# uguryagmur/RealTimeObjectDetection

Hardware: AMD Instinct MI355X
Metric: frames/sec YOLOv3 608x608 bs=8 (Darknet.forward + write_results; 2 batches in flight, write_results_async on a second stream) (higher is better)
Workload: dtype f16x2-split (3 MFMA products, f32 accumulate); 1 GPU; YOLOv3 cfg 608x608 batch=8 per GPU, split-f16 MFMA conv + fused head + GPU NMS (BASELINE configs[2]); precision=f16s3, tiles=autotune (this run), parallelism=frame-shard x1, in_flight_batches=2, detections_last_step=1699, candidates_last_step=1914, f16_range_overflow=False

## Files before the change

realtimeobjectdetection_amd/csrc/conv_f16s3_common.h:

```cpp
#pragma once
#include "rtod_internal.h"
#include <type_traits>

namespace rtod {

typedef float f32x4 __attribute__((ext_vector_type(4)));
typedef _Float16 f16x8 __attribute__((ext_vector_type(8)));
typedef unsigned int u32x4 __attribute__((ext_vector_type(4)));

constexpr int HBK = 32;
constexpr unsigned OOB = 0x80000000u;


template <int N> __device__ __forceinline__ void vmcnt() {
    static_assert(0 <= N && N <= 63, "vmcnt range");
    asm volatile("s_waitcnt vmcnt(%0)" :: "n"(N) : "memory");
}

template <int OFF = 0> __device__ __forceinline__ u32x4 buffer_load_b128(const __amdgpu_buffer_rsrc_t rsrc, unsigned voffset, unsigned soffset) {
    u32x4 v;
    asm volatile("buffer_load_dwordx4 %0, %1, %2, %3 offen offset:%4" : "=v"(v) : "v"(voffset), "s"(rsrc), "s"(soffset), "n"(OFF) : "memory");
    return v;
}

// ... 169 lines not shown
        if (kg == 1) return;
#pragma unroll
        for (int i = 0; i < TM; ++i)
#pragma unroll
            for (int j = 0; j < TN; ++j) {
                const f32x4 o = T[base + (i * TN + j) * 64];
#pragma unroll
                for (int e = 0; e < 4; ++e) acc[i][j][e] += o[e];
            }
    }
    float amax = 0.f;
    _Float16* const oh = reinterpret_cast<_Float16*>(a.out) + a.out_coff;
    const _Float16* const rh = reinterpret_cast<const _Float16*>(a.res) + a.res_coff;
#pragma unroll
    for (int P = 0; P < NP; ++P) {
        const int c0 = cbase + 32 * P + 8 * lh;
        const bool cok = c0 < a.Cout;
        const int cc = cok ? c0 : 0;
        f16x8 rq_h[RES ? TM : 1], rq_l[RES ? TM : 1];
        if constexpr (RES) {
#pragma unroll
            for (int i = 0; i < TM; ++i) {
                const int m = mrow[i];
                const bool ok = m >= 0 && cok;
                const _Float16* q = rh + (int64_t)(ok ? m : 0) * 2 * a.res_ldc + cc;
                rq_h[i] = ok ? *reinterpret_cast<const f16x8*>(q) : f16x8{0, 0, 0, 0, 0, 0, 0, 0};
                rq_l[i] = ok ? *reinterpret_cast<const f16x8*>(q + a.res_ldc) : f16x8{0, 0, 0, 0, 0, 0, 0, 0};
            }
        }
        f32x4 iv0 = *reinterpret_cast<const f32x4*>(a.inv_scale + cc), iv1 = *reinterpret_cast<const f32x4*>(a.inv_scale + cc + 4);
        f32x4 bs0 = *reinterpret_cast<const f32x4*>(a.bias + cc), bs1 = *reinterpret_cast<const f32x4*>(a.bias + cc + 4);
#pragma unroll
        for (int i = 0; i < TM; ++i) {
            const int m = mrow[i];
            f16x8 ph, pl;
#pragma unroll
            for (int e = 0; e < 8; ++e) {
                const float s = e < 4 ? acc[i][2 * P][e] : acc[i][2 * P + 1][e - 4];
                float v = s * ((e < 4 ? iv0[e] : iv1[e - 4]) * SPLIT_SCALE) + (e < 4 ? bs0[e] : bs1[e - 4]) * SPLIT_SCALE;
                if (a.leaky) v = v > 0.f ? v : v * 0.1f;
                if constexpr (RES) v += (float)rq_h[i][e] + (float)rq_l[i][e];
                _Float16 h, l;
                split_f16(v, h, l, amax);
                ph[e] = h; pl[e] = l;
            }
            if (m >= 0 && cok) {
                _Float16* q = oh + (int64_t)m * 2 * a.out_ldc + c0;
                store_act16(q, ph, false);
                store_act16(q + a.out_ldc, pl, false);
            }
        }
    }
    split_overflow_report(a.ovf, amax);
}

constexpr int epi_row_group(int bm, int wm, int rg_max) {
    int best = wm;
    for (int r = wm; r <= bm && r <= rg_max; r += wm) if (bm % r == 0) best = r;
    return best;
}


template <int BM, int BN, int WM, int WN, int NT, int EPI, int SMEM_BYTES, int KG = 1, bool PRE = false, bool F16 = false, bool RAW = false>
__device__ __forceinline__ void conv_f16s3_epilogue(const ConvArgs& a, f32x4 (&acc)[WM / 16][WN / 16], unsigned char* smem,
                                                    int bm, int bn, int tid, int wm, int wn, int lr, int lh, int M, int kg = 0,
                                                    const float* pre_bias = nullptr, const float* pre_inv = nullptr) {
    constexpr int MT = 16, TM = WM / MT, TN = WN / MT;
    constexpr bool PW = EPI == EPI_SPLIT_PW || EPI == EPI_SPLIT_RES_PW;
    constexpr bool RES = EPI == EPI_SPLIT_RES || EPI == EPI_SPLIT_RES_PW;
    static_assert(!(F16 && PW), "plain-f16 plans host no pointwise conv");
    static_assert(!RAW || (EPI == EPI_SPLIT && !F16), "raw-sum instances: no shortcut, decode, hosted pointwise conv or plain-f16 store");
    constexpr int TS = PW ? BN + 4 : BN;
    constexpr int T2S = PW_MAX_COUT + 4;
    constexpr int RG_MAX = SMEM_BYTES / ((TS + (PW ? T2S : 0)) * 4);
    constexpr int RG = epi_row_group(BM, WM, RG_MAX);
    static_assert(RG >= WM && BM % RG == 0, "epilogue row group");
    static_assert(RG * (TS + (PW ? T2S : 0)) * 4 <= SMEM_BYTES, "epilogue tile exceeds the kernel's LDS");
    float* T = reinterpret_cast<float*>(smem);
    const int hw = a.Ho * a.Wo;
#ifdef RTOD_DIAG
    const bool st_plain = (a.dbg & 8) != 0;
#else
    constexpr bool st_plain = false;
#endif
    float amax = 0.f;
    constexpr int PWK = PW_MAX_K / 32;
    f16x8 b2h[PW ? PWK : 1], b2l[PW ? PWK : 1];
    float bias2 = 0.f, inv2 = 0.f;
    int pw_n2t = 1, pw_j = 0;
    if constexpr (PW) {
        pw_n2t = a.pw_cout / 16;
        pw_j = (tid >> 6) % pw_n2t;
        const int n2 = pw_j * 16 + (tid & 15);
        const _Float16* w2h = a.pw_wh + (int64_t)n2 * 32 + ((tid & 63) >> 4) * 8;
        const _Float16* w2l = a.pw_wl + (int64_t)n2 * 32 + ((tid & 63) >> 4) * 8;
#pragma unroll
        for (int ks = 0; ks < PWK; ++ks) {
            const bool ok = ks * 32 < a.pw_k;
            b2h[ks] = ok ? *reinterpret_cast<const f16x8*>(w2h + (int64_t)ks * a.pw_npad * 32) : f16x8{0, 0, 0, 0, 0, 0, 0, 0};
            b2l[ks] = ok ? *reinterpret_cast<const f16x8*>(w2l + (int64_t)ks * a.pw_npad * 32) : f16x8{0, 0, 0, 0, 0, 0, 0, 0};
        }
        bias2 = a.pw_bias[n2] * SPLIT_SCALE; inv2 = a.pw_inv_scale[n2] * SPLIT_SCALE;
    }
    const float escale = (EPI == EPI_DECODE || RAW) ? 1.0f : SPLIT_SCALE;
    constexpr int GPR_ = BN / 8;
    constexpr int NG = (RG * GPR_ + NT - 1) / NT;
#pragma unroll 1
    for (int rg = 0; rg < BM; rg += RG) {
        float bias_j[TN], inv_j[TN];
#pragma unroll
        for (int j = 0; j < TN; ++j) {
            if constexpr (PRE) { bias_j[j] = pre_bias[j]; inv_j[j] = pre_inv[j]; }
            else epi_col_params(a, bn * BN + wn * WN + j * MT + lr, bias_j[j], inv_j[j]);
        }
        f16x8 rq_h[RES ? NG : 1], rq_l[RES ? NG : 1];
        if constexpr (RES) {
            const _Float16* rh0 = reinterpret_cast<const _Float16*>(a.res) + a.res_coff + bn * BN;
#pragma unroll
            for (int i = 0; i < NG; ++i) {
                const int g = tid + i * NT;
                const int r = g / GPR_, c8 = (g - r * GPR_) * 8;
                const int m = bm * BM + rg + r;
                const bool ok = g < RG * GPR_ && m < M && bn * BN + c8 < a.Cout;
                const _Float16* q = rh0 + (int64_t)(ok ? m : 0) * 2 * a.res_ldc + (ok ? c8 : 0);
                const f16x8 th = *reinterpret_cast<const f16x8*>(q);
                rq_h[i] = ok ? th : f16x8{0, 0, 0, 0, 0, 0, 0, 0};
                if constexpr (!F16) {
                    const f16x8 tl = *reinterpret_cast<const f16x8*>(q + a.res_ldc);
                    rq_l[i] = ok ? tl : f16x8{0, 0, 0, 0, 0, 0, 0, 0};
                }
            }
        }
#define EPI_WAVE_IN_PASS (RG == BM || (wm * WM >= rg && wm * WM < rg + RG))
#define EPI_TILE_IN_PASS(i) true
#define EPI_TILE_ROW(i) (wm * WM - rg + (i) * MT)
#include "conv_f16s3_epi_transpose.inc"
#undef EPI_WAVE_IN_PASS
#undef EPI_TILE_IN_PASS
#undef EPI_TILE_ROW
        __syncthreads();
        if constexpr (EPI == EPI_DECODE) {
            constexpr int RSTEP = NT / BN > 0 ? NT / BN : 1;
            static_assert(NT % BN == 0 || BN % NT == 0, "decode mapping");
            for (int nl = tid % BN; nl < BN; nl += NT) {
                const int n = bn * BN + nl;
                if (n >= a.Cout) continue;
                const int an = n / a.dec.attrs, c = n - an * a.dec.attrs;
                const bool is_wh = (c == 2 || c == 3) && !a.dec.train;
                const bool is_raw = (c == 2 || c == 3) && a.dec.train;
                const float anc = (c == 2 ? a.dec.aw[an] : a.dec.ah[an]);
                const int r0 = (NT >= BN) ? tid / BN : 0;
                int m = bm * BM + rg + r0;
                const int b = m / hw;
                int cell = m - b * hw;
                int gy = cell / a.dec.GW, gx = cell - gy * a.dec.GW;
                float* op = a.out + (int64_t)b * a.dec.img_stride + a.dec.head_off + (int64_t)cell * a.Cout + n;
                const int64_t row_step = (int64_t)RSTEP * a.Cout;
                const int64_t img_fix = a.dec.img_stride - (int64_t)hw * a.Cout;
                if (a.dec.v5) {
                    for (int r = r0; r < RG && m < M; r += RSTEP, m += RSTEP) {
                        const float sg = __builtin_amdgcn_rcpf(1.0f + __expf(-T[r * TS + nl]));
                        float o = sg;
                        if (c < 2) o = ((sg * 2.0f - 0.5f) + (float)(c == 0 ? gx : gy)) * a.dec.stride;
                        else if (c < 4) { const float t2 = sg * 2.0f; o = (t2 * t2) * anc; }
                        *op = o;
                        op += row_step; cell += RSTEP; gx += RSTEP;
                        while (gx >= a.dec.GW) { gx -= a.dec.GW; ++gy; }
                        while (cell >= hw) { cell -= hw; gy -= a.dec.GH; op += img_fix; }
                    }
                } else
                for (int r = r0; r < RG && m < M; r += RSTEP, m += RSTEP) {
                    const float v = T[r * TS + nl];
                    float o;
                    if (is_raw) o = v;
                    else {
                        const float ex = __expf(is_wh ? v : -v);
                        if (is_wh) o = (ex * anc) * a.dec.stride;
                        else {
                            o = __builtin_amdgcn_rcpf(1.0f + ex);
                            if (c < 2 && !a.dec.train) o = (o + (float)(c == 0 ? gx : gy)) * a.dec.stride;
                        }
                    }
                    *op = o;
                    op += row_step; cell += RSTEP; gx += RSTEP;
                    while (gx >= a.dec.GW) { gx -= a.dec.GW; ++gy; }
                    while (cell >= hw) { cell -= hw; gy -= a.dec.GH; op += img_fix; }
                }
            }
        } else {
            constexpr int GPR = GPR_;
            _Float16* oh = reinterpret_cast<_Float16*>(a.out) + a.out_coff + bn * BN;
#pragma unroll
            for (int gi = 0; gi < NG; ++gi) {
                const int g = tid + gi * NT;
                if (g >= RG * GPR) continue;
                const int r = g / GPR, c8 = (g - r * GPR) * 8;
                const int m = bm * BM + rg + r;
                if (m >= M || bn * BN + c8 >= a.Cout) continue;
                const f32x4 v0 = *reinterpret_cast<const f32x4*>(T + r * TS + c8);
                const f32x4 v1 = *reinterpret_cast<const f32x4*>(T + r * TS + c8 + 4);
                if constexpr (RAW) {
                    float* rp = a.raw_out + (int64_t)m * a.raw_ld + bn * BN + c8;
                    *reinterpret_cast<f32x4*>(rp) = v0;
                    *reinterpret_cast<f32x4*>(rp + 4) = v1;
                    continue;
                }
                float v[8] = {v0[0], v0[1], v0[2], v0[3], v1[0], v1[1], v1[2], v1[3]};
                if constexpr (RES) {
                    epi_add_shortcut8<F16>(v, rq_h[gi], rq_l[gi]);
                    if constexpr (PW) {
                        *reinterpret_cast<f32x4*>(T + r * TS + c8) = f32x4{v[0], v[1], v[2], v[3]};
                        *reinterpret_cast<f32x4*>(T + r * TS + c8 + 4) = f32x4{v[4], v[5], v[6], v[7]};
                    }
                }
                f16x8 ph, pl;
                epi_split8<F16>(v, ph, pl, amax);
                epi_store8<F16>(oh + (int64_t)m * 2 * a.out_ldc + c8, a.out_ldc, ph, pl, st_plain);
            }
            if constexpr (PW) {
                __syncthreads();
                float* T2 = T + RG * TS;
                const int lane = tid & 63, wave = tid >> 6;
                const int lr16 = lane & 15, lh16 = lane >> 4;
                const int k2s = a.pw_k / 32;
                const int n2 = pw_j * 16 + lr16;
                for (int sl = wave / pw_n2t; sl < RG / 16; sl += (NT / 64) / pw_n2t) {
                    f32x4 acc2 = {0.f, 0.f, 0.f, 0.f};
                    const float* trow = T + (sl * 16 + lr16) * TS + lh16 * 8;
#pragma unroll
                    for (int ks = 0; ks < PWK; ++ks) {
                        if (ks < k2s) {
                            const f32x4 x0 = *reinterpret_cast<const f32x4*>(trow + ks * 32);
                            const f32x4 x1 = *reinterpret_cast<const f32x4*>(trow + ks * 32 + 4);
                            f16x8 ah, al;
#pragma unroll
                            for (int e = 0; e < 8; ++e) {
                                const float x = e < 4 ? x0[e] : x1[e - 4];
                                const _Float16 h = (_Float16)x;
                                ah[e] = h; al[e] = (_Float16)(x - (float)h);
                            }
                            acc2 = __builtin_amdgcn_mfma_f32_16x16x32_f16(al, b2h[ks], acc2, 0, 0, 0);
// ... 39 lines not shown
```

realtimeobjectdetection_amd/csrc/conv_pwd_f16s3.hip:

```cpp
#include "conv_bandd_common.h"

namespace rtod {

template <int BM, int NW, int NST, int MINW, int EPI>
__global__ __launch_bounds__(NW * 64, MINW)
void conv_pwd_f16s3_kernel(const ConvArgs a, const int grid_m, const int grid_n) {
    constexpr bool F16 = epi_f16(EPI);
    constexpr int LB = F16 ? 2 : 4, LP = F16 ? 1 : 2;
    constexpr int BN = NW * 32, NT = NW * 64, TM = BM / 16, TN = 2;
    constexpr int SLAB = BM * 256;
    constexpr int NP = BM / 8;
    constexpr int NPP = (NP + NW - 1) / NW;
    static_assert(BM % 16 == 0 && NPP >= 1 && NPP <= 8, "slab pieces per wave");
    static_assert(NST >= 2 && NST <= 4, "ring depth");
    constexpr int RG = BM * BN * 4 <= 32768 ? BM : (BM / 2) * BN * 4 <= 32768 ? BM / 2 : BM / 4;
    constexpr int WAIT_B = 2 * LB + LP * NPP;
    constexpr int WAIT_SLAB = 2 * LB + (NST - 2) * (LP * NPP + 2 * LB);
    constexpr int WAIT_SLAB_PRO = 2 * LB + (NST - 2) * LP * NPP;

    extern __shared__ __attribute__((aligned(16))) unsigned char smem[];
    const int nwg = grid_m * grid_n;
    int bid = blockIdx.x;
    if (!a.xcd_by_n) bid = xcd_remap(bid, nwg);
    const int bm = bid / grid_n, bn = bid - bm * grid_n;
    const int tid = (int)threadIdx.x;
    const int wave = __builtin_amdgcn_readfirstlane(tid >> 6), lane = tid & 63;
    const int lr = lane & 15, lh = lane >> 4;
    const int M = a.B * a.Hi * a.Wi;
    const int m0 = bm * BM;
    const unsigned PS = (unsigned)a.in_ldc * 4u;
    const unsigned lo_plane = (unsigned)a.in_ldc * 2u;

    const __amdgpu_buffer_rsrc_t rs_a = buffer_rsrc(a.in, a.in_bytes);
    const __amdgpu_buffer_rsrc_t rs_wh = buffer_rsrc(a.w_hi, a.w_bytes);
    const __amdgpu_buffer_rsrc_t rs_wl = buffer_rsrc(a.w_lo, a.w_bytes);
    const unsigned lds0 = (unsigned)(size_t)smem;
    const int NS = a.Cin / 64;

    unsigned dma_vo[NPP];
#pragma unroll
    for (int k = 0; k < NPP; ++k) {
        const int p = wave + k * NW;
        const int r = lane >> 3;
        const int m = m0 + p * 8 + r;
        dma_vo[k] = (p < NP && m < M) ? (unsigned)m * PS + (unsigned)(a.in_coff + (((lane & 7) ^ r) << 3)) * 2u : OOB;
    }
    auto dma_slab = [&](int js) __attribute__((always_inline)) {
        const bool live = js < NS;
        const unsigned soff = (unsigned)js * 128u;
        const unsigned base = lds0 + (unsigned)((js % NST) * SLAB);
#pragma unroll
        for (int k = 0; k < NPP; ++k) {
            const int p = wave + k * NW;
            const unsigned dst = p < NP ? base + (unsigned)((p >> 1) * 4096 + (p & 1) * 1024) : lds0 + (unsigned)(NST * SLAB);
            if constexpr (F16) lds_dma(rs_a, live ? dma_vo[k] : OOB, soff, dst);
// ... 34 lines not shown
        if constexpr (!F16) l = *reinterpret_cast<lds_f16x8*>((unsigned)(o + 4096 * i + 2048));
    };

#pragma unroll
    for (int s = 0; s < NST - 1; ++s) dma_slab(s);
    load_b(0, Bq[0]);
    load_b(1, Bq[1]);

    __builtin_amdgcn_s_setprio(2);
    auto slab_body = [&](int j, auto par_c) __attribute__((always_inline)) {
        constexpr int par = decltype(par_c)::value;
        asm volatile("" : "+v"(xq0), "+v"(xq1));
        if (j < NST - 1) vmcnt<WAIT_SLAB_PRO>(); else vmcnt<WAIT_SLAB>();
        __builtin_amdgcn_sched_barrier(0);
        __builtin_amdgcn_s_barrier();
        dma_slab(j + NST - 1);
        const int slotoff = (int)lds0 + (j % NST) * SLAB;
        read_unit(0, 0, slotoff, Ah[0], Al[0]);
        read_unit(1 / TM, 1 % TM, slotoff, Ah[1], Al[1]);
        __builtin_amdgcn_sched_barrier(0);
#pragma unroll
        for (int u = 0; u < 2 * TM; ++u) {
            const int q = u / TM, i = u % TM;
            if (i == 0) {
                if (q == 0) load_b(2 * j + 2, Bq[(2 * par + 2) % 4]); else load_b(2 * j + 3, Bq[(2 * par + 3) % 4]);
                vmcnt<WAIT_B>();
                if (q == 0) tie_bset<F16>(Bq[2 * par]); else tie_bset<F16>(Bq[2 * par + 1]);
                __builtin_amdgcn_sched_barrier(0);
            }
            if (u + 2 < 2 * TM) read_unit((u + 2) / TM, (u + 2) % TM, slotoff, Ah[(u + 2) % 3], Al[(u + 2) % 3]);
            const f16x8 ah = Ah[u % 3], al = Al[u % 3];
#pragma unroll
            for (int jn = 0; jn < TN; ++jn) {
                const f16x8 bh = __builtin_bit_cast(f16x8, Bq[2 * par + q][jn][0]);
                if constexpr (F16) { acc[i][jn] = __builtin_amdgcn_mfma_f32_16x16x32_f16(ah, bh, acc[i][jn], 0, 0, 0); continue; }
                const f16x8 bl = __builtin_bit_cast(f16x8, Bq[2 * par + q][jn][1]);
                acc[i][jn] = __builtin_amdgcn_mfma_f32_16x16x32_f16(al, bh, acc[i][jn], 0, 0, 0);
                acc[i][jn] = __builtin_amdgcn_mfma_f32_16x16x32_f16(ah, bl, acc[i][jn], 0, 0, 0);
                acc[i][jn] = __builtin_amdgcn_mfma_f32_16x16x32_f16(ah, bh, acc[i][jn], 0, 0, 0);
            }
            __builtin_amdgcn_sched_barrier(0);
        }
    };
#pragma unroll 1
    for (int j = 0; j < NS; j += 2) {
        slab_body(j, std::integral_constant<int, 0>{});
        if (j + 1 < NS) slab_body(j + 1, std::integral_constant<int, 1>{});
    }
    vmcnt<0>();
    tie_bset<F16>(Bq[0]); tie_bset<F16>(Bq[1]); tie_bset<F16>(Bq[2]); tie_bset<F16>(Bq[3]);
    __builtin_amdgcn_sched_barrier(0);
    __builtin_amdgcn_s_setprio(0);

    bandd_epilogue<BM, BN, BM, 32, NT, RG, epi_kind(EPI) == EPI_SPLIT_RES, 1, F16, epi_raw(EPI)>(a, acc, smem, bm, bn, tid, 0, wn, lr, lh, M, 0);
}

template <int BM, int NW, int NST, int MINW>
static int launch_pwd(const ConvArgs& a, hipStream_t s) {
    constexpr int BN = NW * 32, NT = NW * 64;
    constexpr int RG = BM * BN * 4 <= 32768 ? BM : (BM / 2) * BN * 4 <= 32768 ? BM / 2 : BM / 4;
    const int M = a.B * a.Ho * a.Wo;
    const int gm = (M + BM - 1) / BM, gn = (a.Cout + BN - 1) / BN;
    ConvArgs ax = a;
    ax.xcd_by_n = (gn % 8 == 0 && (int64_t)a.Cout * a.K > (int64_t)M * a.Cin) ? 1 : 0;
    constexpr int ring_bytes = NST * BM * 256 + ((BM / 8) % NW ? 4096 : 0), epi_bytes = RG * BN * 4;
    constexpr int lds = ring_bytes > epi_bytes ? ring_bytes : epi_bytes;
    static_assert(lds <= 160 * 1024, "LDS");
    const int fe = a.f16 ? 1 : 0;
    auto k_res = fe ? conv_pwd_f16s3_kernel<BM, NW, NST, MINW, EPI_SPLIT_RES | EPI_F16> : conv_pwd_f16s3_kernel<BM, NW, NST, MINW, EPI_SPLIT_RES>;
    auto k_plain = fe ? conv_pwd_f16s3_kernel<BM, NW, NST, MINW, EPI_SPLIT | EPI_F16> : conv_pwd_f16s3_kernel<BM, NW, NST, MINW, EPI_SPLIT>;
    auto k_raw = conv_pwd_f16s3_kernel<BM, NW, NST, MINW, EPI_SPLIT | EPI_RAW>;
    if constexpr (lds > 64 * 1024) {
        static std::atomic<unsigned long long> attr_done[3] = {{0}, {0}, {0}};
        if (a.raw_out) { if (int rc = lds_opt_in(attr_done[2], lds, "conv_pwd_f16s3", k_raw)) return rc; }
        else if (int rc = lds_opt_in(attr_done[fe], lds, "conv_pwd_f16s3", k_res, k_plain)) return rc;
    }
    if (a.raw_out) {
        hipLaunchKernelGGL(k_raw, dim3(gm * gn), dim3(NT), lds, s, ax, gm, gn);
        return hip_fail(hipGetLastError(), "conv_pwd_f16s3 launch");
    }
    if (a.res) hipLaunchKernelGGL(k_res, dim3(gm * gn), dim3(NT), lds, s, ax, gm, gn);
    else hipLaunchKernelGGL(k_plain, dim3(gm * gn), dim3(NT), lds, s, ax, gm, gn);
    return hip_fail(hipGetLastError(), "conv_pwd_f16s3 launch");
}

#define RTOD_PWD_TILES(X) \
    X(0, 64, 4, 3, 3) X(1, 32, 4, 3, 3) X(2, 128, 4, 3, 1) X(3, 64, 8, 3, 1) X(4, 64, 4, 2, 3) X(5, 32, 4, 4, 3) X(6, 96, 4, 2, 3) X(7, 96, 4, 3, 2) X(8, 48, 4, 3, 3) X(9, 48, 4, 4, 3) X(10, 64, 2, 2, 4)

#define RTOD_X_INFO(idx, bm, nw, nst, minw) {bm, nw * 32, "conv_pwd_f16s3<" #bm "x" #nw "w,r" #nst ">"},
static const ConvVariantInfo kPwdModes[PWD_MODES] = { RTOD_PWD_TILES(RTOD_X_INFO) };
#undef RTOD_X_INFO
const ConvVariantInfo& conv_pwd_mode_info(int idx) { return kPwdModes[idx < 0 || idx >= PWD_MODES ? 0 : idx]; }

bool conv_pwd_supported(int ksize, int stride, int pad, int cin) { return ksize == 1 && stride == 1 && pad == 0 && cin >= 64 && cin % 64 == 0; }

int conv_pwd_kernel_name(int idx, int epi, char* buf, size_t len) {
#define RTOD_X_NAME(i, bm, nw, nst, minw) \
    if (idx == i) return snprintf(buf, len, "void rtod::conv_pwd_f16s3_kernel<" #bm ", " #nw ", " #nst ", " #minw ", %d>(rtod::ConvArgs, int, int)", epi);
    RTOD_PWD_TILES(RTOD_X_NAME)
#undef RTOD_X_NAME
    return -1;
}

int launch_conv_pwd_f16s3(const ConvArgs& a, int idx, hipStream_t s) {
    if (int rc = check_split_conv_args(a, "launch_conv_pwd", true)) return rc;
    if (!conv_pwd_supported(a.kh, a.stride, a.pad, a.Cin) || a.kw != 1 || a.Ho != a.Hi || a.Wo != a.Wi || a.dec.enabled || a.pw_wh) {
        set_error("launch_conv_pwd: unsupported shape (k=%d s=%d pad=%d Cin=%d)", a.kh, a.stride, a.pad, a.Cin); return RTOD_E_ARG;
    }
    if (a.in_ldc % 8 || a.in_coff % 8 || a.K != a.Kpad || a.K != a.Cin || a.Npad % 128) { set_error("launch_conv_pwd: bad view / K"); return RTOD_E_ARG; }
    if (a.raw_out && (a.f16 || a.res)) { set_error("launch_conv_pwd: a raw-sum launch carries no shortcut and no plain-f16 store"); return RTOD_E_ARG; }
    if (a.raw_out && a.raw_ld != a.Npad) { set_error("launch_conv_pwd: raw-sum rows are Npad floats in this family (raw_ld %d, Npad %d)", a.raw_ld, a.Npad); return RTOD_E_ARG; }
    switch (idx) {
#define RTOD_X_CASE(i, bm, nw, nst, minw) case i: return launch_pwd<bm, nw, nst, minw>(a, s);
        RTOD_PWD_TILES(RTOD_X_CASE)
#undef RTOD_X_CASE
    }
    set_error("launch_conv_pwd: mode %d unsupported", idx);
    return RTOD_E_ARG;
}

}
```

realtimeobjectdetection_amd/csrc/plan_tiles.cpp:

```cpp
#include "plan.h"

#include <algorithm>
#include <mutex>

namespace rtod {

int Plan::choose_variant(const Layer& L, int batch) const {
    if (opt_force_f32_variant >= 0 && opt_force_f32_variant < CV_COUNT) return opt_force_f32_variant;
    if (L.cout <= 32) return CV_128x32;
    if (L.cout <= 64) return CV_128x64;
    const int64_t M = (int64_t)batch * L.hout * L.wout;
    const int64_t big = ((M + 127) / 128) * ((L.cout + 127) / 128);
    return big >= 512 ? CV_128x128 : CV_64x64;
}

int Plan::f32_slice_mode(const Launch& l, int batch, int variant) const {
    const PackedConv& pc = convs[l.conv_slot];
    if (pc.split || pc.stem || pc.slice_chunks <= 0) return 0;
    const Layer& L = layers[l.layer];
    const ConvVariantInfo& vi = conv_variant_info(variant);
    const int64_t M = (int64_t)batch * L.hout * L.wout;
    const int64_t tiles = ((M + vi.bm - 1) / vi.bm) * ((L.cout + vi.bn - 1) / vi.bn);
    const int64_t S = (pc.Kpad / 32 + pc.slice_chunks - 1) / pc.slice_chunks;
    return (opt_k_slice_workgroups && d_scratch && tiles < 512 && S * M * pc.Npad <= scratch_floats) ? 2 : 1;
}

bool Plan::tile_legal(const Launch& l, int v) const {
    const TileRef t = family_of(v);
    if (!t || l.kind != LK_CONV || l.conv_slot < 0 || !convs[l.conv_slot].split) return false;
    const PackedConv& pc = convs[l.conv_slot];
    const Layer& L = layers[l.layer];
    if (precision == 2 && !t.f16()) return false;
    if (raw_launch(l) && !t.raw()) return false;
    if (pc.narrow || t.is(TF_C16)) return pc.narrow && t.is(TF_C16);
    if (pc.ks_chunks > 0 || t.is(TF_KS)) return pc.ks_chunks > 0 && t.is(TF_KS);
    if (pc.band) return t.is(TF_BAND) && conv_band_mode_valid(t.mode, L.cin, L.hin, L.win);
    const bool hosts_pw = form(&l - &launches[0]).guest >= 0, plain = l.out_layer != -2 && !hosts_pw, same_map = L.hout == L.hin && L.wout == L.win;
    switch (t.fam->id) {
        case TF_GENERIC: return !(hosts_pw && t.fam->info(t.mode).bn < L.cout);
        case TF_BAND: return t.bandd_wide() && opt_band_kernel && plain && same_map && pc.Npad % 128 == 0 && pc.K == pc.Kpad &&
                             conv_bandd_wide_supported(L.size, L.stride, L.pad, pc.cin_p, L.win);
        case TF_RING: return !hosts_pw && L.act <= 1;
        case TF_PWD: return opt_pwd_kernel && plain && same_map && conv_pwd_supported(L.size, L.stride, L.pad, pc.cin_p);
        case TF_PATCH: return plain && L.act <= 1 && L.hout == L.hin && conv_patch_supported(L.size, L.stride, L.pad, L.cin, L.cout) &&
                              conv_patch_mode_valid(t.mode, L.cin, L.cout);
    }
    return false;
}

int Plan::default_tile(const Launch& l, int batch) const {
    const PackedConv& pc = convs[l.conv_slot];
    const Layer& L = layers[l.layer];
    const int64_t M = (int64_t)batch * L.hout * L.wout;
    if (pc.narrow) return tile_id(TF_C16, conv_c16_default_mode(L.cout, M));
    if (pc.ks_chunks > 0) return tile_id(TF_KS, ((M + 63) / 64) * ((L.cout + 63) / 64) < 512 ? 1 : 0);
    if (pc.band) {
        if (precision != 2 && !raw_launch(l)) return tile_id(TF_BAND, conv_band_default_mode(L.cin, L.hin, L.win));
        const TileFamily& B = tile_family(TF_BAND);
        for (int m = 0; m < B.modes; ++m) if (tile_legal(l, B.base + m)) return B.base + m;
        return B.base + B.f16_from;
    }
    const int64_t gn = (L.cout + 127) / 128;
    const int g = L.cout <= 64 ? HV_128x64 : ((M + 127) / 128) * gn >= 512 ? HV_128x128 : ((M + 63) / 64) * gn >= 512 ? HV_64x128 : HV_64x64;
    return tile_legal(l, g) ? g : HV_128x128_8W;
}

int Plan::variant_for(const Launch& l, int batch) const {
    int want = opt_force_f16s3_variant;
    if (want < 0) {
        auto it = tuned.find(batch);
        const size_t idx = &l - &launches[0];
        if (it != tuned.end() && idx < it->second.size()) want = it->second[idx];
    }
    int v = want >= 0 && tile_legal(l, want) ? want : default_tile(l, batch);
    if (family_of(v).ks_sched_b() && !(opt_k_slice_workgroups && ks_sched_b_fits(l, batch))) --v;
    return v;
}

std::vector<int> Plan::tile_candidates(const Launch& l, int batch) const {
    static const int kOrder[TF_COUNT] = {TF_GENERIC, TF_PATCH, TF_BAND, TF_PWD, TF_RING, TF_C16, TF_KS};
    const int cout = layers[l.layer].cout;
    const bool ks_b = opt_k_slice_workgroups && ks_sched_b_fits(l, batch);
    std::vector<int> cand;
    for (int f : kOrder) {
        if ((f == TF_RING && !opt_ring_kernel) || (f == TF_PATCH && !opt_patch_kernel)) continue;
        const TileFamily& F = tile_family(f);
        for (int m = 0; m < F.modes; ++m) {
            const int bn = F.info(m).bn;
            const bool too_wide = f == TF_GENERIC || f == TF_RING ? bn > 64 && bn > 2 * ((cout + 63) / 64 * 64)
                                : f == TF_PATCH ? bn > 64 && bn > cout
                                : f == TF_PWD ? bn > 128 && bn > (cout + 127) / 128 * 128 : false;
            if (too_wide || (family_of(F.base + m).ks_sched_b() && !ks_b) || !tile_legal(l, F.base + m)) continue;
            cand.push_back(F.base + m);
        }
    }
    return cand;
}

int Plan::launch_split_variant(ConvArgs& a, const PackedConv& pc, int v, hipStream_t s) const {
    const TileRef t = family_of(v);
    if (!t) { set_error("variant %d is no split-f16 tile", v); return RTOD_E_STATE; }
    if (precision == 2 && !t.f16()) { set_error("variant %d has no plain-f16 instance", v); return RTOD_E_STATE; }
    if (a.raw_out && !t.raw()) { set_error("variant %d has no raw-sum instance", v); return RTOD_E_STATE; }
    if (pc.narrow != t.is(TF_C16)) {
        set_error(pc.narrow ? "variant %d requested for a narrow (Cin = 16) layer" : "narrow variant %d requested for a layer without tap-major weights", v);
        return RTOD_E_STATE;
    }
    if ((pc.ks_chunks > 0) != t.is(TF_KS)) {
        set_error(pc.ks_chunks > 0 ? "variant %d requested for a K-sliced layer" : "K-sliced variant %d requested for a layer that is not sliced", v);
        return RTOD_E_STATE;
    }
    if (pc.band != t.is(TF_BAND) && !(t.bandd_wide() && !pc.band)) {
        set_error(pc.band ? "variant %d requested for a band layer" : "band variant %d requested for a layer without band weights", v);
        return RTOD_E_STATE;
    }
    if (t.is(TF_KS)) {
        a.slice_chunks = pc.ks_chunks;
        a.partial = nullptr; a.partial_floats = 0;
        if (t.ks_sched_b()) { a.partial = d_scratch; a.partial_floats = scratch_floats; }
    }
    return t.fam->launch(a, t.mode, s);
}

static std::mutex g_tune_mutex;
static std::map<std::vector<int>, int> g_tune_memo;

int Plan::tune_launch(size_t li, ConvArgs& a, int batch, hipStream_t s) {
    const Launch& l = launches[li];
    const Layer& L = layers[l.layer];
    const bool pw = a.pw_wh != nullptr;
    const std::vector<int> key = {L.cin, L.cout, L.size, L.stride, L.hout, L.wout, l.in2_layer >= 0, l.out_layer == -2, pw ? a.pw_cout : 0,
                                  convs[l.conv_slot].band ? 1 : 0, opt_ring_kernel ? 1 : 0, opt_patch_kernel ? 1 : 0, opt_pwd_kernel ? 1 : 0, L.act,
                                  precision, L.hin, L.win, L.pad, convs[l.conv_slot].ks_chunks, opt_k_slice_workgroups ? 1 : 0,
                                  a.raw_out ? 1 : 0};
    auto it = tune_cache.find(key);
    if (it != tune_cache.end()) { tuning[li] = it->second; return RTOD_OK; }
    std::vector<int> gkey = key; gkey.push_back(device); gkey.push_back(batch);
    {
        std::lock_guard<std::mutex> lock(g_tune_mutex);
        auto git = g_tune_memo.find(gkey);
        if (git != g_tune_memo.end()) { tuning[li] = git->second; tune_cache[key] = git->second; return RTOD_OK; }
    }
    hipEvent_t e0, e1;
    RTOD_HIP(hipEventCreate(&e0)); RTOD_HIP(hipEventCreate(&e1));
// ... 70 lines not shown
```

realtimeobjectdetection_amd/csrc/rtod_internal.h:

```cpp
#pragma once
#include <hip/hip_runtime.h>
#if defined(RTOD_STAMPS) && !defined(RTOD_DIAG)
#define RTOD_DIAG 1
#endif
#include <algorithm>
#include <atomic>
#include <cstdint>
#include <cstdio>
#include <string>
#include <vector>

#include "../../include/rtod.h"

namespace rtod {

void set_error(const char* fmt, ...);
int hip_fail(hipError_t e, const char* what);

#define RTOD_HIP(expr)                                              \
    do {                                                            \
        hipError_t _e = (expr);                                     \
        if (_e != hipSuccess) return ::rtod::hip_fail(_e, #expr);   \
    } while (0)

// ... 129 lines not shown
constexpr int BANDD_WIDE_MODE = BAND_LDS_MODES + 7;
bool conv_bandd_wide_supported(int ksize, int stride, int pad, int cin, int w_in);
int conv_bandd_kernel_name(int idx, int epi, char* buf, size_t len);
int launch_conv_bandd_f16s3(const ConvArgs& a, int idx, hipStream_t s);
int conv_band_layer_kg(int cin, int h, int w);
bool conv_band_mode_valid(int mode, int cin, int h, int w);
int conv_band_default_mode(int cin, int h, int w);
const ConvVariantInfo& conv_band_mode_info(int mode);
int conv_band_kernel_name(int mode, int epi, char* buf, size_t len);
int launch_conv_band_f16s3(const ConvArgs& a, int mode, hipStream_t s);
constexpr int BAND_VARIANT_BASE = 50;
constexpr int RING_MODES = 8;
constexpr int RING_VARIANT_BASE = 70;
const ConvVariantInfo& conv_ring_mode_info(int mode);
int conv_ring_kernel_name(int mode, int epi, char* buf, size_t len);
int launch_conv_ring_f16s3(const ConvArgs& a, int mode, hipStream_t s);
constexpr int PWD_MODES = 11;
constexpr int PWD_VARIANT_BASE = 90;
bool conv_pwd_supported(int ksize, int stride, int pad, int cin);
const ConvVariantInfo& conv_pwd_mode_info(int mode);
int conv_pwd_kernel_name(int mode, int epi, char* buf, size_t len);
int launch_conv_pwd_f16s3(const ConvArgs& a, int mode, hipStream_t s);
constexpr int STEM2_VARIANT = 130;
bool conv_stem2_supported(int k0, int s0, int p0, int cin0, int cout0, int k1, int s1, int p1, int cout1, int pw_cout);
int conv_stem2_kernel_name(int pw, char* buf, size_t len);
int launch_conv_stem2_f16s3(const float* x, int B, int H, int W, const _Float16* w0h, const _Float16* w0l, const float* inv0, const float* bias0,
                            int leaky0, const ConvArgs& c1, hipStream_t s);
constexpr int PATCH_MODES = 5;
constexpr int PATCH_WRES_MODE = 4;
bool conv_patch_mode_valid(int mode, int cin, int cout);
constexpr int PATCH_VARIANT_BASE = 110;
bool conv_patch_supported(int ksize, int stride, int pad, int cin, int cout);
const ConvVariantInfo& conv_patch_mode_info(int mode);
int conv_patch_kernel_name(int mode, int epi, char* buf, size_t len);
int launch_conv_patch_f16s3(const ConvArgs& a, int mode, hipStream_t s);

constexpr int C16_MODES = 4;
constexpr int C16_VARIANT_BASE = 140;
constexpr bool conv_c16_supported(int cin) { return cin == 16; }
const ConvVariantInfo& conv_c16_mode_info(int mode);
int conv_c16_default_mode(int cout, int64_t m);
int conv_c16_kernel_name(int mode, int epi, char* buf, size_t len);
int launch_conv_c16_f16s3(const ConvArgs& a, int mode, hipStream_t s);

constexpr int KS_TILES = 3;
constexpr int KS_MODES = 2 * KS_TILES;
constexpr int KS_VARIANT_BASE = 150;
constexpr int64_t KS_SCRATCH_FLOATS = 8ll << 20;
const ConvVariantInfo& conv_ks_mode_info(int mode);
int conv_ks_slices(const ConvArgs& a);
int conv_ks_kernel_name(int mode, int epi, char* buf, size_t len);
int launch_conv_ks_f16s3(const ConvArgs& a, int mode, hipStream_t s);

enum TileFamilyId { TF_GENERIC = 0, TF_BAND, TF_RING, TF_PWD, TF_PATCH, TF_C16, TF_KS, TF_COUNT };
struct TileFamily {
    int id, base, modes;
    int f16_from;
    int raw_from;
    const ConvVariantInfo& (*info)(int mode);
    int (*kernel_name)(int mode, int epi, char* buf, size_t len);
    int (*launch)(const ConvArgs& a, int mode, hipStream_t s);
};
struct TileRef {
    const TileFamily* fam; int mode;
    explicit operator bool() const { return fam != nullptr; }
    bool is(int family) const { return fam && fam->id == family; }
    bool f16() const { return fam && mode >= fam->f16_from; }
    bool raw() const { return fam && mode >= fam->raw_from; }
    bool ks_sched_b() const { return is(TF_KS) && (mode & 1); }
    bool bandd_wide() const { return is(TF_BAND) && mode == BANDD_WIDE_MODE; }
};
TileRef family_of(int v);
const TileFamily& tile_family(int family);
inline int tile_id(int family, int mode) { return tile_family(family).base + mode; }

int launch_conv_stem(const float* x_nchw, const float* w, const float* bias, const View& out, int B, int H, int W,
                     int Ho, int Wo, int stride, int Cout, int leaky, hipStream_t s);
int launch_conv_stem_split(const float* x_nchw, const _Float16* wh, const _Float16* wl, const float* inv_scale, const float* bias,
                           const View& out, int B, int H, int W, int Ho, int Wo, int stride, int Cout, int leaky, int32_t* ovf, hipStream_t s);
bool conv_stem16_supported(int ksize, int stride, int pad, int cin, int cout, int act);
int launch_conv_stem16_f16s3(const float* x_nchw, const _Float16* wh, const _Float16* wl, const float* inv_scale, const float* bias,
                             const View& out, int B, int H, int W, int act, int pool, int32_t* ovf, hipStream_t s);
int launch_conv_stem16_raw(const float* x_nchw, const _Float16* wh, const _Float16* wl, const float* inv_scale, const View& raw, int B, int H, int W, hipStream_t s);
int launch_prep_image(const unsigned char* img, int h, int w, int bgr, int inp_dim, float* out, hipStream_t s);
int launch_prep_frames(const unsigned char* frames, int batch, int h, int w, int bgr, int out_h, int out_w, float* out, hipStream_t s);
int launch_pack_input(const float* x_nchw, int B, int C, int H, int W, float* out_nhwc, int Cp, hipStream_t s);
int launch_upsample2x(const View& in, const View& out, int B, hipStream_t s);
int launch_add(const View& a, const View& b, const View& out, int B, hipStream_t s, int32_t* ovf = nullptr);
int launch_maxpool(const View& in, const View& out, int B, int size, int stride, int pad, hipStream_t s);
int launch_upsample_nearest2x(const View& in, const View& out, int B, hipStream_t s);
int launch_bn_batch(const View& x, const View& y, const View* res, int B, double* stats, int sstride, const float* bn, int gstride, int act,
                    double* partial, int64_t partial_doubles, hipStream_t s);
size_t bn_partial_doubles(int max_channels);
int launch_bn_batch_split(const View& raw, const View& y, const View* res, int B, double* stats, int sstride, const float* bn, int gstride, int act,
                          double* partial, int64_t partial_doubles, int32_t* ovf, hipStream_t s, int pool = 0);
struct BnUpdateEntry { float* running_mean; float* running_var; int64_t stats_off; double unbias; int sstride; int channels; };
constexpr int BN_UPDATE_MAX = 32;
struct BnUpdateTable { BnUpdateEntry e[BN_UPDATE_MAX]; };
int launch_bn_update_running(const BnUpdateEntry* entries, int n, const double* stats, double momentum, hipStream_t s);
int launch_copy(const View& in, const View& out, int B, hipStream_t s);
int launch_view_to_nchw(const View& in, int B, float* out_nchw, hipStream_t s);
int launch_finish_decode(float* out, int B, const DecodeArgs& d, int hw_exp, hipStream_t s);
int launch_decode(const float* raw, int64_t sb, int64_t sc, int64_t sy, int64_t sx, int B,
                  const DecodeArgs& d, float* out, hipStream_t s);
int launch_confidence_mask(const float* pred, int64_t rows, int attrs, float conf, float* out, hipStream_t s);
int launch_bbox_iou(const float* box1, const float* boxes, int k, int row_stride, float* iou, hipStream_t s);

// ... 57 lines not shown
```

realtimeobjectdetection_amd/csrc/split_tiles.cpp:

```cpp
#include "rtod_internal.h"

namespace rtod {

static const TileFamily kFamilies[TF_COUNT] = {
    {TF_GENERIC, 0, HV_COUNT, 0, 0, conv_f16s3_variant_info, conv_f16s3_kernel_name, launch_conv_f16s3},
    {TF_BAND, BAND_VARIANT_BASE, BAND_MODES, BAND_LDS_MODES, BAND_LDS_MODES, conv_band_mode_info, conv_band_kernel_name, launch_conv_band_f16s3},
    {TF_RING, RING_VARIANT_BASE, RING_MODES, RING_MODES, RING_MODES, conv_ring_mode_info, conv_ring_kernel_name, launch_conv_ring_f16s3},
    {TF_PWD, PWD_VARIANT_BASE, PWD_MODES, 0, 0, conv_pwd_mode_info, conv_pwd_kernel_name, launch_conv_pwd_f16s3},
    {TF_PATCH, PATCH_VARIANT_BASE, PATCH_MODES, PATCH_MODES, PATCH_MODES, conv_patch_mode_info, conv_patch_kernel_name, launch_conv_patch_f16s3},
    {TF_C16, C16_VARIANT_BASE, C16_MODES, 0, 0, conv_c16_mode_info, conv_c16_kernel_name, launch_conv_c16_f16s3},
    {TF_KS, KS_VARIANT_BASE, KS_MODES, 0, KS_MODES, conv_ks_mode_info, conv_ks_kernel_name, launch_conv_ks_f16s3},
};
static_assert(HV_COUNT <= BAND_VARIANT_BASE, "generic tile ids end where the band family's begin");
static_assert(BAND_VARIANT_BASE + BAND_MODES <= RING_VARIANT_BASE, "band tile ids end where the ring family's begin");
static_assert(RING_VARIANT_BASE + RING_MODES <= PWD_VARIANT_BASE, "ring tile ids end where the pwd family's begin");
static_assert(PWD_VARIANT_BASE + PWD_MODES <= PATCH_VARIANT_BASE, "pwd tile ids end where the patch family's begin");
static_assert(PATCH_VARIANT_BASE + PATCH_MODES <= STEM2_VARIANT && STEM2_VARIANT < C16_VARIANT_BASE, "the fused stem's reported id lies between the patch and narrow families");
static_assert(C16_VARIANT_BASE + C16_MODES <= KS_VARIANT_BASE, "narrow tile ids end where the K-sliced family's begin");

TileRef family_of(int v) {
    for (const TileFamily& f : kFamilies)
        if (v >= f.base && v < f.base + f.modes) return {&f, v - f.base};
    return {nullptr, 0};
}

const TileFamily& tile_family(int family) { return kFamilies[family]; }

}
```

Baseline: 2582 frames/s.

## Add pointwise-conv decode tile family and vectorize YOLO decode epilogue stores

Adds a new tile family that runs the YOLO detection-head 1x1 convs through the pointwise (pwd) kernel with the box-decode epilogue fused in, so the autotuner can pick it for head layers. It also rewrites the decode epilogue so each thread handles four adjacent channels, uses branchless per-element selection, and realigns outputs with lane shuffles to issue 16-byte vector stores instead of scalar ones. The aim is cheaper head convs and wider, coalesced global writes of decoded detections. The cost is more kernel instances, more complex alignment and edge handling in the store path, and reliance on the autotuner choosing the new tiles.

```diff
diff --git a/realtimeobjectdetection_amd/csrc/conv_f16s3_common.h b/realtimeobjectdetection_amd/csrc/conv_f16s3_common.h
--- a/realtimeobjectdetection_amd/csrc/conv_f16s3_common.h
+++ b/realtimeobjectdetection_amd/csrc/conv_f16s3_common.h
@@ -245,6 +245,83 @@
         }
     }
     split_overflow_report(a.ovf, amax);
+}
+
+template <int BN, int NT, int TS>
+__device__ __forceinline__ void epi_decode_tile(const ConvArgs& a, const float* T, int n0, int m0, int rows, int M, int tid) {
+    constexpr int TPR = BN / 4;
+    static_assert(BN % 4 == 0 && TS % 4 == 0 && TPR >= 1 && TPR <= 64 && (TPR & (TPR - 1)) == 0 && NT % 64 == 0, "decode mapping");
+    constexpr int RSTEP = NT / TPR;
+    const int hw = a.Ho * a.Wo;
+    const int j = tid % TPR, r0 = tid / TPR;
+    float anc[4]; bool is_x[4], is_xy[4], is_wh[4];
+#pragma unroll
+    for (int e = 0; e < 4; ++e) {
+        const int n = n0 + 4 * j + e < a.Cout ? n0 + 4 * j + e : 0;
+        const int an = n / a.dec.attrs, c = n - an * a.dec.attrs;
+        is_x[e] = c == 0; is_xy[e] = c < 2; is_wh[e] = c == 2 || c == 3;
+        anc[e] = (c == 2 ? a.dec.aw[an] : a.dec.ah[an]);
+    }
+    int m = m0 + r0;
+    const int b = m / hw;
+    int cell = m - b * hw;
+    int gy = cell / a.dec.GW, gx = cell - gy * a.dec.GW;
+    float* op = a.out + (int64_t)b * a.dec.img_stride + a.dec.head_off + (int64_t)cell * a.Cout + n0;
+    const int64_t row_step = (int64_t)RSTEP * a.Cout;
+    const int64_t img_fix = a.dec.img_stride - (int64_t)hw * a.Cout;
+    const int src = ((tid & 63) & ~(TPR - 1)) | ((j + TPR - 1) & (TPR - 1));
+    for (int r = r0; r - r0 < rows; r += RSTEP, m += RSTEP) {
+        const bool live = r < rows && m < M;
+        const f32x4 t = *reinterpret_cast<const f32x4*>(T + (live ? r : 0) * TS + 4 * j);
+        const float gxf = (float)gx, gyf = (float)gy;
+        float o[4];
+        if (a.dec.v5) {
+#pragma unroll
+            for (int e = 0; e < 4; ++e) {
+                const float sg = __builtin_amdgcn_rcpf(1.0f + __expf(-t[e]));
+                const float xy = ((sg * 2.0f - 0.5f) + (is_x[e] ? gxf : gyf)) * a.dec.stride;
+                const float t2 = sg * 2.0f;
+                const float wh = (t2 * t2) * anc[e];
+                o[e] = is_xy[e] ? xy : is_wh[e] ? wh : sg;
+            }
+        } else if (a.dec.train) {
+#pragma unroll
+            for (int e = 0; e < 4; ++e) {
+                const float sg = __builtin_amdgcn_rcpf(1.0f + __expf(-t[e]));
+                o[e] = is_wh[e] ? t[e] : sg;
+            }
+        } else {
+#pragma unroll
+            for (int e = 0; e < 4; ++e) {
+                const float v = t[e];
+                const float ex = __expf(is_wh[e] ? v : -v);
+                const float wh = (ex * anc[e]) * a.dec.stride;
+                const float sg = __builtin_amdgcn_rcpf(1.0f + ex);
+                const float xy = (sg + (is_x[e] ? gxf : gyf)) * a.dec.stride;
+                o[e] = is_wh[e] ? wh : is_xy[e] ? xy : sg;
+            }
+        }
+        const float p1 = __shfl(o[1], src), p2 = __shfl(o[2], src), p3 = __shfl(o[3], src);
+        const int d = (int)((reinterpret_cast<uintptr_t>(op) >> 2) & 3);
+        const f32x4 w = {d == 0 ? o[0] : d == 1 ? p3 : d == 2 ? p2 : p1,
+                         d == 0 ? o[1] : d == 1 ? o[0] : d == 2 ? p3 : p2,
+                         d == 0 ? o[2] : d == 1 ? o[1] : d == 2 ? o[0] : p3,
+                         d == 0 ? o[3] : d == 1 ? o[2] : d == 2 ? o[1] : o[0]};
+        const int ch0 = 4 * j - d;
+        if (live) {
+            if (ch0 >= 0 && n0 + ch0 + 3 < a.Cout) *reinterpret_cast<f32x4*>(op + ch0) = w;
+            else {
+#pragma unroll
+                for (int e = 0; e < 4; ++e) {
+                    const int ch = ch0 + e < 0 ? ch0 + e + BN : ch0 + e;
+                    if (n0 + ch < a.Cout) op[ch] = w[e];
+                }
+            }
+        }
+        op += row_step; cell += RSTEP; gx += RSTEP;
+        while (gx >= a.dec.GW) { gx -= a.dec.GW; ++gy; }
+        while (cell >= hw) { cell -= hw; gy -= a.dec.GH; op += img_fix; }
+    }
 }
 
 constexpr int epi_row_group(int bm, int wm, int rg_max) {
@@ -270,7 +347,6 @@
     static_assert(RG >= WM && BM % RG == 0, "epilogue row group");
     static_assert(RG * (TS + (PW ? T2S : 0)) * 4 <= SMEM_BYTES, "epilogue tile exceeds the kernel's LDS");
     float* T = reinterpret_cast<float*>(smem);
-    const int hw = a.Ho * a.Wo;
 #ifdef RTOD_DIAG
     const bool st_plain = (a.dbg & 8) != 0;
 #else
@@ -333,53 +409,7 @@
 #undef EPI_TILE_ROW
         __syncthreads();
         if constexpr (EPI == EPI_DECODE) {
-            constexpr int RSTEP = NT / BN > 0 ? NT / BN : 1;
-            static_assert(NT % BN == 0 || BN % NT == 0, "decode mapping");
-            for (int nl = tid % BN; nl < BN; nl += NT) {
-                const int n = bn * BN + nl;
-                if (n >= a.Cout) continue;
-                const int an = n / a.dec.attrs, c = n - an * a.dec.attrs;
-                const bool is_wh = (c == 2 || c == 3) && !a.dec.train;
-                const bool is_raw = (c == 2 || c == 3) && a.dec.train;
-                const float anc = (c == 2 ? a.dec.aw[an] : a.dec.ah[an]);
-                const int r0 = (NT >= BN) ? tid / BN : 0;
-                int m = bm * BM + rg + r0;
-                const int b = m / hw;
-                int cell = m - b * hw;
-                int gy = cell / a.dec.GW, gx = cell - gy * a.dec.GW;
-                float* op = a.out + (int64_t)b * a.dec.img_stride + a.dec.head_off + (int64_t)cell * a.Cout + n;
-                const int64_t row_step = (int64_t)RSTEP * a.Cout;
-                const int64_t img_fix = a.dec.img_stride - (int64_t)hw * a.Cout;
-                if (a.dec.v5) {
-                    for (int r = r0; r < RG && m < M; r += RSTEP, m += RSTEP) {
-                        const float sg = __builtin_amdgcn_rcpf(1.0f + __expf(-T[r * TS + nl]));
-                        float o = sg;
-                        if (c < 2) o = ((sg * 2.0f - 0.5f) + (float)(c == 0 ? gx : gy)) * a.dec.stride;
-                        else if (c < 4) { const float t2 = sg * 2.0f; o = (t2 * t2) * anc; }
-                        *op = o;
-                        op += row_step; cell += RSTEP; gx += RSTEP;
-                        while (gx >= a.dec.GW) { gx -= a.dec.GW; ++gy; }
-                        while (cell >= hw) { cell -= hw; gy -= a.dec.GH; op += img_fix; }
-                    }
-                } else
-                for (int r = r0; r < RG && m < M; r += RSTEP, m += RSTEP) {
-                    const float v = T[r * TS + nl];
-                    float o;
-                    if (is_raw) o = v;
-                    else {
-                        const float ex = __expf(is_wh ? v : -v);
-                        if (is_wh) o = (ex * anc) * a.dec.stride;
-                        else {
-                            o = __builtin_amdgcn_rcpf(1.0f + ex);
-                            if (c < 2 && !a.dec.train) o = (o + (float)(c == 0 ? gx : gy)) * a.dec.stride;
-                        }
-                    }
-                    *op = o;
-                    op += row_step; cell += RSTEP; gx += RSTEP;
-                    while (gx >= a.dec.GW) { gx -= a.dec.GW; ++gy; }
-                    while (cell >= hw) { cell -= hw; gy -= a.dec.GH; op += img_fix; }
-                }
-            }
+            epi_decode_tile<BN, NT, TS>(a, T, bn * BN, bm * BM + rg, RG, M, tid);
         } else {
             constexpr int GPR = GPR_;
             _Float16* oh = reinterpret_cast<_Float16*>(a.out) + a.out_coff + bn * BN;
diff --git a/realtimeobjectdetection_amd/csrc/conv_pwd_f16s3.hip b/realtimeobjectdetection_amd/csrc/conv_pwd_f16s3.hip
--- a/realtimeobjectdetection_amd/csrc/conv_pwd_f16s3.hip
+++ b/realtimeobjectdetection_amd/csrc/conv_pwd_f16s3.hip
@@ -1,6 +1,29 @@
 #include "conv_bandd_common.h"
 
 namespace rtod {
+
+template <int BM, int BN, int NT>
+__device__ __forceinline__ void pwd_decode_epilogue(const ConvArgs& a, f32x4 (&acc)[BM / 16][2], unsigned char* smem, int bm, int bn, int tid,
+                                                    int wn, int lr, int lh, int M) {
+    constexpr int TM = BM / 16, TN = 2, MT = 16, TS = BN, WN = 32, KG = 1;
+    constexpr bool RAW = false;
+    constexpr int kg = 0;
+    float* T = reinterpret_cast<float*>(smem);
+    const float escale = 1.0f;
+    float bias_j[TN], inv_j[TN];
+#pragma unroll
+    for (int j = 0; j < TN; ++j) epi_col_params(a, bn * BN + wn * WN + j * MT + lr, bias_j[j], inv_j[j]);
+    __syncthreads();
+#define EPI_WAVE_IN_PASS true
+#define EPI_TILE_IN_PASS(i) true
+#define EPI_TILE_ROW(i) ((i) * MT)
+#include "conv_f16s3_epi_transpose.inc"
+#undef EPI_WAVE_IN_PASS
+#undef EPI_TILE_IN_PASS
+#undef EPI_TILE_ROW
+    __syncthreads();
+    epi_decode_tile<BN, NT, TS>(a, T, bn * BN, bm * BM, BM, M, tid);
+}
 
 template <int BM, int NW, int NST, int MINW, int EPI>
 __global__ __launch_bounds__(NW * 64, MINW)
@@ -141,6 +164,10 @@
     __builtin_amdgcn_sched_barrier(0);
     __builtin_amdgcn_s_setprio(0);
 
+    if constexpr (epi_kind(EPI) == EPI_DECODE) {
+        static_assert(!F16 && !epi_raw(EPI), "decode instances: f16s3 only");
+        pwd_decode_epilogue<BM, BN, NT>(a, acc, smem, bm, bn, tid, wn, lr, lh, M);
+    } else
     bandd_epilogue<BM, BN, BM, 32, NT, RG, epi_kind(EPI) == EPI_SPLIT_RES, 1, F16, epi_raw(EPI)>(a, acc, smem, bm, bn, tid, 0, wn, lr, lh, M, 0);
 }
 
@@ -191,6 +218,60 @@
     return -1;
 }
 
+template <int BM, int NW, int NST, int MINW>
+static int launch_pwd_dec(const ConvArgs& a, hipStream_t s) {
+    constexpr int BN = NW * 32, NT = NW * 64;
+    const int M = a.B * a.Ho * a.Wo;
+    const int gm = (M + BM - 1) / BM, gn = (a.Cout + BN - 1) / BN;
+    ConvArgs ax = a;
+    ax.xcd_by_n = 0;
+    constexpr int ring_bytes = NST * BM * 256 + ((BM / 8) % NW ? 4096 : 0), epi_bytes = BM * BN * 4;
+    constexpr int lds = ring_bytes > epi_bytes ? ring_bytes : epi_bytes;
+    static_assert(lds <= 64 * 1024, "LDS without the opt-in");
+    hipLaunchKernelGGL((conv_pwd_f16s3_kernel<BM, NW, NST, MINW, EPI_DECODE>), dim3(gm * gn), dim3(NT), lds, s, ax, gm, gn);
+    return hip_fail(hipGetLastError(), "conv_pwd_f16s3 decode launch");
+}
+
+#define RTOD_PWD_DEC_TILES(X) \
+    X(0, 64, 8, 3, 1) X(1, 32, 8, 3, 2) X(2, 96, 4, 2, 3) X(3, 64, 4, 3, 3) X(4, 48, 4, 3, 3) X(5, 32, 4, 3, 3)
+
+#define RTOD_X_INFO(idx, bm, nw, nst, minw) {bm, nw * 32, "conv_pwd_f16s3<" #bm "x" #nw "w,r" #nst ",decode>"},
+static const ConvVariantInfo kPwdDecModes[PWD_DEC_MODES] = { RTOD_PWD_DEC_TILES(RTOD_X_INFO) };
+#undef RTOD_X_INFO
+const ConvVariantInfo& conv_pwd_dec_mode_info(int idx) { return kPwdDecModes[idx < 0 || idx >= PWD_DEC_MODES ? 0 : idx]; }
+
+int conv_pwd_dec_kernel_name(int idx, int epi, char* buf, size_t len) {
+#define RTOD_X_NAME(i, bm, nw, nst, minw) \
+    if (idx == i) return snprintf(buf, len, "void rtod::conv_pwd_f16s3_kernel<" #bm ", " #nw ", " #nst ", " #minw ", %d>(rtod::ConvArgs, int, int)", epi);
+    RTOD_PWD_DEC_TILES(RTOD_X_NAME)
+#undef RTOD_X_NAME
+    return -1;
+}
+
+int launch_conv_pwd_dec_f16s3(const ConvArgs& a, int idx, hipStream_t s) {
+    if (int rc = check_split_conv_args(a, "launch_conv_pwd_dec", false)) return rc;
+    if (!conv_pwd_supported(a.kh, a.stride, a.pad, a.Cin) || a.kw != 1 || a.Ho != a.Hi || a.Wo != a.Wi || a.pw_wh || a.res || a.raw_out || a.f16) {
+        set_error("launch_conv_pwd_dec: unsupported launch (k=%d s=%d pad=%d Cin=%d; f16s3 head convs without shortcut, raw sums or hosted conv)", a.kh, a.stride, a.pad, a.Cin);
+        return RTOD_E_ARG;
+    }
+    if (a.in_ldc % 8 || a.in_coff % 8 || a.K != a.Kpad || a.K != a.Cin || a.Npad % 128 || a.Cout <= 0 || a.Cout > a.Npad) { set_error("launch_conv_pwd_dec: bad view / K"); return RTOD_E_ARG; }
+    if (a.B <= 0 || a.Ho <= 0 || a.Wo <= 0 || (int64_t)a.B * a.Ho * a.Wo >= (1ll << 31) - 256) { set_error("launch_conv_pwd_dec: empty or oversized shape"); return RTOD_E_ARG; }
+    const DecodeArgs& d = a.dec;
+    if (!d.enabled || d.attrs < 5 || d.n_anchors < 1 || d.n_anchors > 4 || d.n_anchors * d.attrs != a.Cout || d.GH != a.Ho || d.GW != a.Wo ||
+        d.head_off < 0 || d.img_stride < d.head_off + (int64_t)a.Ho * a.Wo * a.Cout) {
+        set_error("launch_conv_pwd_dec: decode arguments do not describe this conv (enabled %d, %d anchors x %d attributes for %d channels, grid %dx%d for %dx%d)",
+                  d.enabled, d.n_anchors, d.attrs, a.Cout, d.GH, d.GW, a.Ho, a.Wo);
+        return RTOD_E_ARG;
+    }
+    switch (idx) {
+#define RTOD_X_CASE(i, bm, nw, nst, minw) case i: return launch_pwd_dec<bm, nw, nst, minw>(a, s);
+        RTOD_PWD_DEC_TILES(RTOD_X_CASE)
+#undef RTOD_X_CASE
+    }
+    set_error("launch_conv_pwd_dec: mode %d unsupported", idx);
+    return RTOD_E_ARG;
+}
+
 int launch_conv_pwd_f16s3(const ConvArgs& a, int idx, hipStream_t s) {
     if (int rc = check_split_conv_args(a, "launch_conv_pwd", true)) return rc;
     if (!conv_pwd_supported(a.kh, a.stride, a.pad, a.Cin) || a.kw != 1 || a.Ho != a.Hi || a.Wo != a.Wi || a.dec.enabled || a.pw_wh) {
diff --git a/realtimeobjectdetection_amd/csrc/plan_tiles.cpp b/realtimeobjectdetection_amd/csrc/plan_tiles.cpp
--- a/realtimeobjectdetection_amd/csrc/plan_tiles.cpp
+++ b/realtimeobjectdetection_amd/csrc/plan_tiles.cpp
@@ -44,6 +44,8 @@
         case TF_PWD: return opt_pwd_kernel && plain && same_map && conv_pwd_supported(L.size, L.stride, L.pad, pc.cin_p);
         case TF_PATCH: return plain && L.act <= 1 && L.hout == L.hin && conv_patch_supported(L.size, L.stride, L.pad, L.cin, L.cout) &&
                               conv_patch_mode_valid(t.mode, L.cin, L.cout);
+        case TF_PWD_DEC: return opt_pwd_kernel && l.out_layer == -2 && !hosts_pw && l.in2_layer < 0 && same_map && pc.Npad % 128 == 0 &&
+                                conv_pwd_supported(L.size, L.stride, L.pad, pc.cin_p);
     }
     return false;
 }
@@ -78,7 +80,7 @@
 }
 
 std::vector<int> Plan::tile_candidates(const Launch& l, int batch) const {
-    static const int kOrder[TF_COUNT] = {TF_GENERIC, TF_PATCH, TF_BAND, TF_PWD, TF_RING, TF_C16, TF_KS};
+    static const int kOrder[TF_COUNT] = {TF_GENERIC, TF_PATCH, TF_BAND, TF_PWD, TF_PWD_DEC, TF_RING, TF_C16, TF_KS};
     const int cout = layers[l.layer].cout;
     const bool ks_b = opt_k_slice_workgroups && ks_sched_b_fits(l, batch);
     std::vector<int> cand;
@@ -89,7 +91,7 @@
             const int bn = F.info(m).bn;
             const bool too_wide = f == TF_GENERIC || f == TF_RING ? bn > 64 && bn > 2 * ((cout + 63) / 64 * 64)
                                 : f == TF_PATCH ? bn > 64 && bn > cout
-                                : f == TF_PWD ? bn > 128 && bn > (cout + 127) / 128 * 128 : false;
+                                : f == TF_PWD || f == TF_PWD_DEC ? bn > 128 && bn > (cout + 127) / 128 * 128 : false;
             if (too_wide || (family_of(F.base + m).ks_sched_b() && !ks_b) || !tile_legal(l, F.base + m)) continue;
             cand.push_back(F.base + m);
         }
diff --git a/realtimeobjectdetection_amd/csrc/rtod_internal.h b/realtimeobjectdetection_amd/csrc/rtod_internal.h
--- a/realtimeobjectdetection_amd/csrc/rtod_internal.h
+++ b/realtimeobjectdetection_amd/csrc/rtod_internal.h
@@ -205,7 +205,13 @@
 int conv_ks_kernel_name(int mode, int epi, char* buf, size_t len);
 int launch_conv_ks_f16s3(const ConvArgs& a, int mode, hipStream_t s);
 
-enum TileFamilyId { TF_GENERIC = 0, TF_BAND, TF_RING, TF_PWD, TF_PATCH, TF_C16, TF_KS, TF_COUNT };
+constexpr int PWD_DEC_MODES = 6;
+constexpr int PWD_DEC_VARIANT_BASE = 170;
+const ConvVariantInfo& conv_pwd_dec_mode_info(int mode);
+int conv_pwd_dec_kernel_name(int mode, int epi, char* buf, size_t len);
+int launch_conv_pwd_dec_f16s3(const ConvArgs& a, int mode, hipStream_t s);
+
+enum TileFamilyId { TF_GENERIC = 0, TF_BAND, TF_RING, TF_PWD, TF_PATCH, TF_C16, TF_KS, TF_PWD_DEC, TF_COUNT };
 struct TileFamily {
     int id, base, modes;
     int f16_from;
diff --git a/realtimeobjectdetection_amd/csrc/split_tiles.cpp b/realtimeobjectdetection_amd/csrc/split_tiles.cpp
--- a/realtimeobjectdetection_amd/csrc/split_tiles.cpp
+++ b/realtimeobjectdetection_amd/csrc/split_tiles.cpp
@@ -10,6 +10,7 @@
     {TF_PATCH, PATCH_VARIANT_BASE, PATCH_MODES, PATCH_MODES, PATCH_MODES, conv_patch_mode_info, conv_patch_kernel_name, launch_conv_patch_f16s3},
     {TF_C16, C16_VARIANT_BASE, C16_MODES, 0, 0, conv_c16_mode_info, conv_c16_kernel_name, launch_conv_c16_f16s3},
     {TF_KS, KS_VARIANT_BASE, KS_MODES, 0, KS_MODES, conv_ks_mode_info, conv_ks_kernel_name, launch_conv_ks_f16s3},
+    {TF_PWD_DEC, PWD_DEC_VARIANT_BASE, PWD_DEC_MODES, PWD_DEC_MODES, PWD_DEC_MODES, conv_pwd_dec_mode_info, conv_pwd_dec_kernel_name, launch_conv_pwd_dec_f16s3},
 };
 static_assert(HV_COUNT <= BAND_VARIANT_BASE, "generic tile ids end where the band family's begin");
 static_assert(BAND_VARIANT_BASE + BAND_MODES <= RING_VARIANT_BASE, "band tile ids end where the ring family's begin");
@@ -17,6 +18,7 @@
 static_assert(PWD_VARIANT_BASE + PWD_MODES <= PATCH_VARIANT_BASE, "pwd tile ids end where the patch family's begin");
 static_assert(PATCH_VARIANT_BASE + PATCH_MODES <= STEM2_VARIANT && STEM2_VARIANT < C16_VARIANT_BASE, "the fused stem's reported id lies between the patch and narrow families");
 static_assert(C16_VARIANT_BASE + C16_MODES <= KS_VARIANT_BASE, "narrow tile ids end where the K-sliced family's begin");
+static_assert(KS_VARIANT_BASE + KS_MODES <= PWD_DEC_VARIANT_BASE, "K-sliced tile ids end where the decode slab family's begin");
 
 TileRef family_of(int v) {
     for (const TileFamily& f : kFamilies)
```

Result: no change. 2589 frames/s, median of 5 (+0.3%).
